# tsinghua-fib-lab/DRL-urban-planning

Measured on NVIDIA H100. Metric: ppo_update_graph_samples_per_sec, higher is better.
Workload: dtype f32

## Files before the change

drl_urban_planning_b200/csrc/sgnn_kernel.cuh:

```cuda
#pragma once
#include <cuda_runtime.h>
#include <math_constants.h>
#include <stdint.h>

#include "blob.h"
#include "layout.h"

namespace upb {

constexpr int NT = 512;
constexpr int NW = NT / 32;
constexpr int NS = 464;
constexpr int AS = 5632;
constexpr int KS = 160;
constexpr int CH = 96;
constexpr float MASK_FILL = -4294967296.0f;
constexpr float EPS_DEG = 1e-6f;

constexpr int S_WET = 0;
constexpr int S_BE = S_WET + 384;
constexpr int S_WPQ0 = S_BE + 16;
constexpr int S_B0 = S_WPQ0 + 512;
constexpr int S_WPQ1 = S_B0 + 16;
constexpr int S_B1 = S_WPQ1 + 512;
// ... 325 lines not shown
    v.z += __shfl_xor_sync(0xffffffffu, v.z, o); v.w += __shfl_xor_sync(0xffffffffu, v.w, o);
    w.x += __shfl_xor_sync(0xffffffffu, w.x, o); w.y += __shfl_xor_sync(0xffffffffu, w.y, o);
    w.z += __shfl_xor_sync(0xffffffffu, w.z, o); w.w += __shfl_xor_sync(0xffffffffu, w.w, o);
  }
  const int lane = threadIdx.x & 31, warp = threadIdx.x >> 5;
  if (lane < 4) { st4(red + warp * 20 + lane * 4, v); }
  __syncthreads();
  float keep = 0.f;
  if (threadIdx.x < 16) {
#pragma unroll
    for (int x = 0; x < NW; ++x) keep += red[x * 20 + threadIdx.x];
  }
  __syncthreads();
  if (lane < 4) { st4(red + warp * 20 + lane * 4, w); }
  if (threadIdx.x < 16) out32[threadIdx.x] = keep;
  __syncthreads();
  if (threadIdx.x < 16) {
    float s = 0.f;
#pragma unroll
    for (int x = 0; x < NW; ++x) s += red[x * 20 + threadIdx.x];
    out32[16 + threadIdx.x] = s;
  }
  __syncthreads();
}
__device__ __forceinline__ void block_sum_q4p1(float4 v, float sc1, float* red, float* out32) {
#pragma unroll
  for (int o = 4; o < 32; o <<= 1) {
    v.x += __shfl_xor_sync(0xffffffffu, v.x, o); v.y += __shfl_xor_sync(0xffffffffu, v.y, o);
    v.z += __shfl_xor_sync(0xffffffffu, v.z, o); v.w += __shfl_xor_sync(0xffffffffu, v.w, o);
  }
  sc1 = warp_sum(sc1);
  const int lane = threadIdx.x & 31, warp = threadIdx.x >> 5;
  if (lane < 4) st4(red + warp * 20 + lane * 4, v);
  if (lane == 0) red[warp * 20 + 16] = sc1;
  __syncthreads();
  if (threadIdx.x < 17) {
    float s = 0.f;
#pragma unroll
    for (int x = 0; x < NW; ++x) s += red[x * 20 + threadIdx.x];
    out32[threadIdx.x] = s;
  }
  __syncthreads();
}

template <bool TANH>
__device__ __forceinline__ void matvec8(const float* __restrict__ W, const float* __restrict__ b, int rows, int cols,
                                        const float* x, float* y) {
  const int p = threadIdx.x & 7;
  for (int row = threadIdx.x >> 3; row < rows; row += NT / 8) {
    const float* w = W + (size_t)row * cols;
    float acc = 0.f;
#pragma unroll 9
    for (int k = p; k < cols; k += 8) acc = fmaf(__ldg(w + k), x[k], acc);
    acc += __shfl_xor_sync(0xffffffffu, acc, 1);
    acc += __shfl_xor_sync(0xffffffffu, acc, 2);
    acc += __shfl_xor_sync(0xffffffffu, acc, 4);
    if (p == 0) {
      acc += __ldg(b + row);
      y[row] = TANH ? tanhf(acc) : acc;
    }
  }
}

__device__ __forceinline__ void load_weights(const float* __restrict__ P, float* sW) {
  const int t = threadIdx.x;
  static_assert(NT == 512, "load_weights is laid out for 512 threads");
  const int o = t >> 4, c = t & 15;
  const int src = o < 16 ? o * 32 + c : (o - 16) * 32 + 16 + c;
  const float wet = (t < 384 && (t >> 4) < F) ? __ldg(P + P_ENC_W + c * F + (t >> 4)) : 0.f;
  const float g0 = __ldg(P + P_GCN0_W + src), g1 = __ldg(P + P_GCN1_W + src);
  const float in0 = __ldg(P + P_MHA_IN_W + t), in1 = t < 256 ? __ldg(P + P_MHA_IN_W + 512 + t) : 0.f;
  float wq = 0.f, wk = 0.f, wv = 0.f, wo = 0.f;
  if (t < 256) {
    wq = __ldg(P + P_ATT_Q_W + t); wk = __ldg(P + P_ATT_K_W + t); wv = __ldg(P + P_ATT_V_W + t);
    wo = __ldg(P + P_MHA_OUT_W + t);
  }
  float lu[4];
#pragma unroll
  for (int j = 0; j < 4; ++j) lu[j] = __ldg(P + P_LU_W0 + t + NT * j);
  const float rd = __ldg(P + P_RD_W0 + t);
  float sm0 = 0.f, sm1 = 0.f, sm2 = 0.f;
  if (t < 16) { sm0 = __ldg(P + P_ENC_B + t); sm1 = __ldg(P + P_GCN0_B + t); sm2 = __ldg(P + P_GCN1_B + t); }
  else if (t < 32) { sm0 = __ldg(P + P_MHA_OUT_B + t - 16); sm1 = __ldg(P + P_ATT_Q_B + t - 16); sm2 = __ldg(P + P_ATT_V_B + t - 16); }
  else if (t < 64) { sm0 = __ldg(P + P_LU_B0 + t - 32); sm1 = __ldg(P + P_LU_W1 + t - 32); }
  else if (t < 96) { sm0 = __ldg(P + P_RD_B0 + t - 64); sm1 = __ldg(P + P_RD_W1 + t - 64); }
  else if (t < 112) { sm0 = __ldg(P + P_MHA_IN_B + t - 96); sm1 = __ldg(P + P_MHA_IN_B + 32 + t - 96); }

  float* tmp = sW + S_EPQ;
  if (t < 384) sW[S_WET + t] = wet;
  sW[S_WPQ0 + t] = g0; sW[S_WPQ1 + t] = g1;
  sW[S_WPQT0 + c * 32 + o] = g0; sW[S_WPQT1 + c * 32 + o] = g1;
  tmp[t] = in0;
  if (t < 256) {
    tmp[512 + t] = in1;
    tmp[768 + t] = wq; tmp[1024 + t] = wk; tmp[1280 + t] = wv;
    sW[S_WO + t] = wo;
    sW[S_WOT + c * 16 + o] = wo;
  }
#pragma unroll
  for (int j = 0; j < 4; ++j) sW[S_LUW0 + t + NT * j] = lu[j];
  sW[S_RDW0 + t] = rd;
  sW[S_RDW0T + c * 32 + o] = rd;
  if (t < 16) { sW[S_BE + t] = sm0; sW[S_B0 + t] = sm1; sW[S_B1 + t] = sm2; }
  else if (t < 32) { sW[S_BO + t - 16] = sm0; tmp[1536 + t - 16] = sm1; tmp[1552 + t - 16] = sm2; }
  else if (t < 64) { sW[S_LUB0 + t - 32] = sm0; sW[S_LUW1 + t - 32] = sm1; }
  else if (t < 96) { sW[S_RDB0 + t - 64] = sm0; sW[S_RDW1 + t - 64] = sm1; }
  else if (t < 112) { tmp[1568 + t - 96] = sm0; tmp[1584 + t - 96] = sm1; }
  __syncthreads();
  if (t < 256) {
    float q = 0.f, k = 0.f, v = 0.f;
#pragma unroll
    for (int m = 0; m < 16; ++m) {
      q = fmaf(tmp[o * 16 + m], tmp[768 + m * 16 + c], q);
      k = fmaf(tmp[(16 + o) * 16 + m], tmp[1024 + m * 16 + c], k);
      v = fmaf(tmp[(32 + o) * 16 + m], tmp[1280 + m * 16 + c], v);
    }
    sW[S_QC + t] = q; sW[S_KC + t] = k; sW[S_VC + t] = v;
    const int tr = c * 16 + o;
    sW[S_QCT + tr] = q; sW[S_KCT + tr] = k; sW[S_VCT + tr] = v;
  } else if (t < 272) {
    const int r = t - 256;
    float q = tmp[1568 + r], v = tmp[1584 + r];
#pragma unroll
    for (int m = 0; m < 16; ++m) {
      q = fmaf(tmp[r * 16 + m], tmp[1536 + m], q);
      v = fmaf(tmp[(32 + r) * 16 + m], tmp[1552 + m], v);
    }
    sW[S_QBC + r] = q;
    sW[S_VBC + r] = v;
  }
}

struct GraphView {
  int n, e, k, stage, gid;
  const float* x;
  float* H0g;
  float* H1g;
  float* EPQ;
  float* GPQ;
  float* H;
  float* inv;
  float* alpha;
  float* z;
  float* gz;
  float* ghead;
  const uint16_t* rp;
  const uint16_t* ord;
  int ord_rounds;
  const uint32_t* adj;
  const uint32_t* cuv;
  const int* cidx;
};

__device__ __forceinline__ uint32_t tf32_of(float x) {
  uint32_t r;
  asm("cvt.rna.tf32.f32 %0, %1;" : "=r"(r) : "f"(x));
  return r;
}
__device__ __forceinline__ void tf32_split(float x, uint32_t& hi, uint32_t& lo) {
  hi = tf32_of(x);
  lo = tf32_of(x - __uint_as_float(hi));
}
__device__ __forceinline__ void mma_tf32(float (&c)[4], uint32_t a0, uint32_t a1, uint32_t a2, uint32_t a3, uint32_t b0,
                                         uint32_t b1) {
  asm volatile("mma.sync.aligned.m16n8k8.row.col.f32.tf32.tf32.f32 {%0,%1,%2,%3}, {%4,%5,%6,%7}, {%8,%9}, {%0,%1,%2,%3};"
               : "+f"(c[0]), "+f"(c[1]), "+f"(c[2]), "+f"(c[3])
               : "r"(a0), "r"(a1), "r"(a2), "r"(a3), "r"(b0), "r"(b1));
}
#ifdef UPB_TILE_BF16
__device__ __forceinline__ uint32_t bf16_round(float x) {
  uint32_t u = __float_as_uint(x);
  u += 0x7fffu + ((u >> 16) & 1u);
  return u & 0xffff0000u;
}
__device__ __forceinline__ void mma_3x(float (&c)[4], float a0, float a1, float a2, float a3, uint32_t bh0, uint32_t bh1,
                                       uint32_t bl0, uint32_t bl1) {
  (void)bl0; (void)bl1;
  mma_tf32(c, bf16_round(a0), bf16_round(a1), bf16_round(a2), bf16_round(a3),
           bf16_round(__uint_as_float(bh0)), bf16_round(__uint_as_float(bh1)));
}
#else
__device__ __forceinline__ void mma_3x(float (&c)[4], float a0, float a1, float a2, float a3, uint32_t bh0, uint32_t bh1,
                                       uint32_t bl0, uint32_t bl1) {
  uint32_t h0, h1, h2, h3, l0, l1, l2, l3;
  tf32_split(a0, h0, l0); tf32_split(a1, h1, l1); tf32_split(a2, h2, l2); tf32_split(a3, h3, l3);
  mma_tf32(c, l0, l1, l2, l3, bh0, bh1);
  mma_tf32(c, h0, h1, h2, h3, bl0, bl1);
  mma_tf32(c, h0, h1, h2, h3, bh0, bh1);
}
#endif

__device__ __forceinline__ void gh_phase_tc(const GraphView& g, const float* Wpq, bool rescale) {
  const int lane = threadIdx.x & 31, warp = threadIdx.x >> 5;
  const int gq = lane >> 2, t = lane & 3;
  uint32_t bh[2][8], bl[2][8];
#pragma unroll
  for (int nt = 0; nt < 2; ++nt)
#pragma unroll
    for (int j = 0; j < 8; ++j) {
      const int k = (j < 4 ? 0 : 16) + 4 * t + (j & 3);
      tf32_split(Wpq[k * 16 + nt * 8 + gq], bh[nt][j], bl[nt][j]);
    }
  const int n = g.n;
  for (int m0 = warp * 16; m0 < n; m0 += NW * 16) {
    const int r0 = min(m0 + gq, n - 1), r1 = min(m0 + gq + 8, n - 1);
    const float4 v0 = ld4(g.GPQ + r0 * 32 + 4 * t), v1 = ld4(g.GPQ + r0 * 32 + 16 + 4 * t);
    const float4 w0 = ld4(g.GPQ + r1 * 32 + 4 * t), w1 = ld4(g.GPQ + r1 * 32 + 16 + 4 * t);
    const float rd0 = (float)(g.rp[r0 + 1] - g.rp[r0]) + EPS_DEG, rd1 = (float)(g.rp[r1 + 1] - g.rp[r1]) + EPS_DEG;
    float acc[2][4];
#pragma unroll
    for (int nt = 0; nt < 2; ++nt) {
      const float2 h0 = *reinterpret_cast<const float2*>(g.H + r0 * 16 + nt * 8 + 2 * t);
      const float2 h1 = *reinterpret_cast<const float2*>(g.H + r1 * 16 + nt * 8 + 2 * t);
      acc[nt][0] = h0.x * rd0; acc[nt][1] = h0.y * rd0; acc[nt][2] = h1.x * rd1; acc[nt][3] = h1.y * rd1;
      mma_3x(acc[nt], v0.x, w0.x, v0.y, w0.y, bh[nt][0], bh[nt][1], bl[nt][0], bl[nt][1]);
      mma_3x(acc[nt], v0.z, w0.z, v0.w, w0.w, bh[nt][2], bh[nt][3], bl[nt][2], bl[nt][3]);
      mma_3x(acc[nt], v1.x, w1.x, v1.y, w1.y, bh[nt][4], bh[nt][5], bl[nt][4], bl[nt][5]);
      mma_3x(acc[nt], v1.z, w1.z, v1.w, w1.w, bh[nt][6], bh[nt][7], bl[nt][6], bl[nt][7]);
    }
    const float s0 = rescale ? g.inv[r0] : 1.f, s1 = rescale ? g.inv[r1] : 1.f;
    __syncwarp();
#pragma unroll
    for (int nt = 0; nt < 2; ++nt) {
      if (m0 + gq < n)
        *reinterpret_cast<float2*>(g.H + (m0 + gq) * 16 + nt * 8 + 2 * t) = make_float2(acc[nt][0] * s0, acc[nt][1] * s0);
      if (m0 + gq + 8 < n)
        *reinterpret_cast<float2*>(g.H + (m0 + gq + 8) * 16 + nt * 8 + 2 * t) = make_float2(acc[nt][2] * s1, acc[nt][3] * s1);
    }
  }
}

template <bool RAW>
__device__ __forceinline__ int epq_phase(const GraphView& g, const float* hsrc, const float* WT, const float* b) {
  const int og = threadIdx.x & 7;
  const float4 bias = og < 4 ? ld4(b + og * 4) : f4(0.f);
  float2 wlo[16], whi[16];
#pragma unroll
  for (int c = 0; c < 16; ++c) {
    const float4 w = ld4(WT + c * 32 + og * 4);
    wlo[c] = make_float2(w.x, w.y); whi[c] = make_float2(w.z, w.w);
  }
  const int npair = (g.n + 1) >> 1;
  float amax = 0.f;
  for (int task = threadIdx.x; task < npair * 8; task += NT) {
    const int i0 = (task >> 3) * 2;
    const int i1 = min(i0 + 1, g.n - 1);
    float4 ha[4], hb[4];
#pragma unroll
    for (int j = 0; j < 4; ++j) { ha[j] = ld4(hsrc + i0 * 16 + j * 4); hb[j] = ld4(hsrc + i1 * 16 + j * 4); }
    float2 a0 = make_float2(bias.x, bias.y), a1 = make_float2(bias.z, bias.w), b0 = a0, b1 = a1;
#pragma unroll
    for (int c = 0; c < 16; ++c) {
      const float xa = comp(ha[c >> 2], c & 3), xb = comp(hb[c >> 2], c & 3);
      const float2 xa2 = make_float2(xa, xa), xb2 = make_float2(xb, xb);
      a0 = ffma2(wlo[c], xa2, a0); a1 = ffma2(whi[c], xa2, a1);
      b0 = ffma2(wlo[c], xb2, b0); b1 = ffma2(whi[c], xb2, b1);
    }
    amax = fmaxf(amax, fmaxf(fmaxf(fabsf(a0.x), fabsf(a0.y)), fmaxf(fabsf(a1.x), fabsf(a1.y))));
    amax = fmaxf(amax, fmaxf(fmaxf(fabsf(b0.x), fabsf(b0.y)), fmaxf(fabsf(b1.x), fabsf(b1.y))));
    if constexpr (RAW) {
      st4(g.EPQ + i0 * 32 + og * 4, make_float4(a0.x, a0.y, a1.x, a1.y));
      if (i1 != i0) st4(g.EPQ + i1 * 32 + og * 4, make_float4(b0.x, b0.y, b1.x, b1.y));
    } else {
      st4(g.EPQ + i0 * 32 + og * 4, make_float4(exp2a(a0.x), exp2a(a0.y), exp2a(a1.x), exp2a(a1.y)));
      if (i1 != i0) st4(g.EPQ + i1 * 32 + og * 4, make_float4(exp2a(b0.x), exp2a(b0.y), exp2a(b1.x), exp2a(b1.y)));
    }
  }
  return !(amax <= 10.9f) + !(amax <= 40.f);
}


template <int TIER, bool SM>
__device__ __forceinline__ void pull_forward(const GraphView& g, int q, bool save_h1, float* h1g, bool want_sums,
                                             float4& msum, float4& hsum) {
  const int odd = (threadIdx.x >> 2) & 1;
  const int offX = (odd ? 16 : 0) + q * 4, offY = (odd ? 0 : 16) + q * 4;
  const RowBase<SM> rX(g.EPQ + offX), rY(g.EPQ + offY);
  for (int task = threadIdx.x; task < g.ord_rounds * NT; task += NT) {
    const int i = g.ord[task >> 2];
    if (i == kNoNode) continue;
    const F2x2 A = rY.row((unsigned)i, 7), B = rX.row((unsigned)i, 7);
    const int beg = g.rp[i], end = g.rp[i + 1];
    float2 s0 = make_float2(0.f, 0.f), s1 = s0, s2 = s0, s3 = s0;
    int t = beg;
    for (; t + 1 < end; t += 2) {
      const unsigned k0 = g.adj[t] & 0xffffu, k1 = g.adj[t + 1] & 0xffffu;
      const F2x2 X0 = rX.row(k0, 7), Y0 = rY.row(k0, 7);
      const F2x2 X1 = rX.row(k1, 7), Y1 = rY.row(k1, 7);
      fwd_term<TIER>(A.a, B.a, Y0.a, X0.a, s0);
      fwd_term<TIER>(A.b, B.b, Y0.b, X0.b, s1);
      fwd_term<TIER>(A.a, B.a, Y1.a, X1.a, s2);
      fwd_term<TIER>(A.b, B.b, Y1.b, X1.b, s3);
    }
    if (t < end) {
      const unsigned k0 = g.adj[t] & 0xffffu;
      const F2x2 X0 = rX.row(k0, 7), Y0 = rY.row(k0, 7);
      fwd_term<TIER>(A.a, B.a, Y0.a, X0.a, s0);
      fwd_term<TIER>(A.b, B.b, Y0.b, X0.b, s1);
    }
    const float cnt = (float)(end - beg);
    const float4 acc = make_float4(cnt - (s0.x + s2.x), cnt - (s0.y + s2.y), cnt - (s1.x + s3.x), cnt - (s1.y + s3.y));
    const float iv = g.inv[i];
    float4 h = ld4(g.H + i * 16 + q * 4);
    h.x = fmaf(acc.x, iv, h.x); h.y = fmaf(acc.y, iv, h.y); h.z = fmaf(acc.z, iv, h.z); h.w = fmaf(acc.w, iv, h.w);
    st4(g.H + i * 16 + q * 4, h);
    if (save_h1) st4(h1g + i * 16 + q * 4, h);
    if (want_sums) { msum = msum + acc; hsum = hsum + h; }
  }
}

template <int TIER, bool SM>
__device__ __forceinline__ float4 pull_backward(const GraphView& g, int q, float4 ce4, bool use_head) {
  float4 bsum = f4(0.f);
  const float2 two = make_float2(2.f, 2.f);
// ... 298 lines not shown
}
__device__ __forceinline__ float half_sum(float v, unsigned mask) {
#pragma unroll
  for (int o = 8; o > 0; o >>= 1) v += __shfl_xor_sync(mask, v, o, 16);
  return v;
}

template <bool TRAIN>
__device__ __forceinline__ void softmax_seeds(const StepArgs& a, const BlobHeader& hd, const GraphView& g, float* sc,
                                              float* stats, int lane) {
  const int k = g.k, gid = g.gid;
  float lmax = -CUDART_INF_F;
  int lbest = 0x7fffffff;
  for (int j = lane; j < k; j += 32) {
    const float zj = g.z[j];
    if (zj > lmax) { lmax = zj; lbest = j; }
  }
#pragma unroll
  for (int o = 16; o > 0; o >>= 1) {
    const float om = __shfl_xor_sync(0xffffffffu, lmax, o);
    const int ob = __shfl_xor_sync(0xffffffffu, lbest, o);
    if (om > lmax || (om == lmax && ob < lbest)) { lmax = om; lbest = ob; }
  }
  const float zmax = lmax;
  float lsum = 0.f;
  for (int j = lane; j < k; j += 32) lsum += expf(g.z[j] - zmax);
  const float lse = zmax + logf(warp_sum(lsum));
  const int aidx = a.actions ? (int)sc[SC_ACT] : -1;
  float lent = 0.f;
  int slot = -1;
  for (int j = lane; j < k; j += 32) {
    const float lp = g.z[j] - lse;
    lent -= expf(lp) * lp;
    if (g.cidx[j] == aidx) slot = j;
  }
#pragma unroll
  for (int o = 16; o > 0; o >>= 1) slot = max(slot, __shfl_xor_sync(0xffffffffu, slot, o));
  float H = warp_sum(lent), logp = 0.f;
  int greedy = 0;
  if (k > 0) {
    greedy = g.cidx[lbest];
    if (a.actions) logp = slot >= 0 ? g.z[slot] - lse : MASK_FILL - lse;
  } else {
    H = 0.f;
    logp = 0.f;
  }
  const float V = sc[SC_VALUE];
  if (lane == 0) {
    sc[SC_LSE] = lse; sc[SC_ENT] = H; sc[SC_LOGP] = logp; sc[SC_SLOT] = (float)(slot + 1);
    if (a.out_value) a.out_value[gid] = V;
    if (a.out_logp) a.out_logp[gid] = logp;
    if (a.out_entropy) a.out_entropy[gid] = H;
    if (a.out_greedy) a.out_greedy[gid] = greedy;
  }
  if constexpr (!TRAIN) {
    if (a.uniforms != nullptr && a.out_sample != nullptr) {
      const float u = a.uniforms[gid];
      int pick = -1;
      if (k > 0) {
        const float S = warp_sum(lsum), target = u * S;
        float run = 0.f;
        int last = -1;
        for (int base = 0; base < k && pick < 0; base += 32) {
          const int j = base + lane;
          const float ej = j < k ? expf(g.z[j] - zmax) : 0.f;
          float c = ej;
#pragma unroll
          for (int o = 1; o < 32; o <<= 1) {
            const float t = __shfl_up_sync(0xffffffffu, c, o);
            if (lane >= o) c += t;
          }
          c += run;
          const unsigned pos = __ballot_sync(0xffffffffu, ej / S > 0.f);
          const unsigned hit = pos & __ballot_sync(0xffffffffu, c > target);
          if (hit) pick = base + __ffs(hit) - 1;
          if (pos) last = base + 31 - __clz(pos);
          run = __shfl_sync(0xffffffffu, c, 31);
        }
        if (pick < 0) pick = last;
        pick = g.cidx[pick];
      } else {
        const int cap = g.stage == 0 ? hd.e_cap : hd.n_cap;
        pick = min(cap - 1, max(0, (int)(u * (float)cap)));
      }
      if (lane == 0) a.out_sample[gid] = pick;
    }
  }
  if constexpr (TRAIN) {
    const float R = sc[SC_RET], dv = V - R;
    float glp = 0.f, gH = 0.f, surr = 0.f, negent = 0.f, in_ind = 0.f, kl = 0.f, clipped = 0.f;
    if (sc[SC_EXP] != 0.f) {
      in_ind = 1.f;
      const float dlp = logp - sc[SC_FLP];
      const float r = expf(dlp), A = sc[SC_ADV];
      const float lo = 1.f - a.clip_eps, hi = 1.f + a.clip_eps;
      const float s1 = r * A, s2 = fminf(fmaxf(r, lo), hi) * A;
      const bool inside = r >= lo && r <= hi;
      surr = -fminf(s1, s2);
      if (inside || s1 < s2) glp = -A * r * a.inv_ind;
      gH = -a.c_entropy * a.inv_ind;
      negent = -H;
      kl = expm1f(dlp) - dlp;
      clipped = inside ? 0.f : 1.f;
    }
    if (lane == 0) {
      sc[SC_GV] = 2.f * a.c_value * dv * a.inv_batch;
      gacc(stats, 0, dv * dv); gacc(stats, 1, surr); gacc(stats, 2, negent); gacc(stats, 3, 1.f); gacc(stats, 4, in_ind);
      gacc(stats, 5, g.stage == 0 ? 1.f : 0.f); gacc(stats, 6, g.stage == 1 ? 1.f : 0.f);
      gacc(stats, 7, (isfinite(V) && isfinite(logp) && isfinite(H)) ? 0.f : 1.f);
      if (a.diagnostics) {
        gacc(stats, 8, kl); gacc(stats, 9, clipped); gacc(stats, 10, R); gacc(stats, 11, R * R); gacc(stats, 12, dv);
      }
    }
    for (int j = lane; j < k; j += 32) {
      const float lp = g.z[j] - lse, p = expf(lp);
      g.gz[j] = glp * ((j == slot ? 1.f : 0.f) - p) - gH * p * (lp + H);
    }
  }
}

template <bool TRAIN>
__device__ __noinline__ void prefetch_next_graph(const StepArgs& a, int nitem) {
  const int T0 = threadIdx.x, TN = NT;
  const BlobHeader& hd = *reinterpret_cast<const BlobHeader*>(a.blob);
  const GraphDesc* descs = reinterpret_cast<const GraphDesc*>(a.blob + hd.off_desc);
  const int ng = a.ids ? a.ids[nitem] : nitem;
  const GraphDesc& nd = descs[ng];
  const char* px = reinterpret_cast<const char*>(a.blob + hd.off_x) + (size_t)nd.x_row * FS * 4;
  const char* pa = reinterpret_cast<const char*>(a.blob + hd.off_adj) + (size_t)nd.adj_off * 4;
  const char* pr = reinterpret_cast<const char*>(a.blob + hd.off_rowptr) + (size_t)nd.rp_off * 2;
  const char* po = reinterpret_cast<const char*>(a.blob + hd.off_order) + (size_t)nd.ord_off * 2;
  const int bx = nd.n * FS * 4, ba = nd.e * 8, br = (nd.n + 1) * 2, bo = nd.ord_rounds * NW * 16;
  for (int o = T0 * 128; o < bx; o += TN * 128) asm volatile("prefetch.global.L2 [%0];" ::"l"(px + o));
  for (int o = T0 * 128; o < ba; o += TN * 128) asm volatile("prefetch.global.L2 [%0];" ::"l"(pa + o));
  for (int o = T0 * 128; o < br; o += TN * 128) asm volatile("prefetch.global.L2 [%0];" ::"l"(pr + o));
  for (int o = T0 * 128; o < bo; o += TN * 128) asm volatile("prefetch.global.L2 [%0];" ::"l"(po + o));
  if (T0 >= TN - 32) {
    const int w = T0 - (TN - 32);
    const void* q = nullptr;
    if (w < 3) q = reinterpret_cast<const char*>(a.blob + hd.off_num) + (size_t)ng * NUMD * 4 + min(w * 128, NUMD * 4 - 4);
    else if (w < 5) q = reinterpret_cast<const char*>(a.blob + hd.off_cur) + (size_t)ng * FS * 4 + (w - 3) * (FS * 4 - 4);
    else if (w == 5) q = a.actions ? a.actions + (size_t)ng * 2 : nullptr;
    else if (TRAIN && w == 6) q = a.ret + ng;
    else if (TRAIN && w == 7) q = a.exps + ng;
    else if (TRAIN && w == 8) q = a.fixed_lp + ng;
    else if (TRAIN && w == 9) q = a.adv + ng;
    if (q) asm volatile("prefetch.global.L2 [%0];" ::"l"(q));
  }
}

template <bool SMEM>
__device__ __forceinline__ void gw_partial(const GraphView& g, const float* hin, int n, float* redbuf) {
  const int lane = threadIdx.x & 31, warp = threadIdx.x >> 5;
  const int to = lane >> 2, tc = lane & 3;
  float2 accp[4][2];
#pragma unroll
  for (int c = 0; c < 4; ++c) { accp[c][0] = make_float2(0.f, 0.f); accp[c][1] = make_float2(0.f, 0.f); }
  for (int i = warp; i < n; i += 8 * KW) {
    float4 gq[8], hv[8];
#pragma unroll
    for (int u = 0; u < 8; ++u) {
      const int ii = i + u * KW;
      if constexpr (SMEM) hv[u] = ii < n ? ld4(hin + ii * 16 + tc * 4) : f4(0.f);
      else hv[u] = ii < n ? __ldcg(reinterpret_cast<const float4*>(hin + (size_t)ii * 16 + tc * 4)) : f4(0.f);
    }
#pragma unroll
    for (int u = 0; u < 8; ++u) {
      const int ii = i + u * KW;
      gq[u] = ii < n ? ld4(g.GPQ + ii * 32 + to * 4) : f4(0.f);
    }
#pragma unroll
    for (int u = 0; u < 8; ++u) {
      const float2 g01 = make_float2(gq[u].x, gq[u].y), g23 = make_float2(gq[u].z, gq[u].w);
#pragma unroll
      for (int c = 0; c < 4; ++c) {
        const float hc_ = comp(hv[u], c);
        const float2 h2 = make_float2(hc_, hc_);
        accp[c][0] = ffma2(g01, h2, accp[c][0]);
        accp[c][1] = ffma2(g23, h2, accp[c][1]);
      }
    }
  }
#pragma unroll
  for (int x = 0; x < 4; ++x) {
    const int xp = x >> 1;
    st4(redbuf + warp * 512 + (to * 4 + x) * 16 + tc * 4,
        (x & 1) ? make_float4(accp[0][xp].y, accp[1][xp].y, accp[2][xp].y, accp[3][xp].y)
                : make_float4(accp[0][xp].x, accp[1][xp].x, accp[2][xp].x, accp[3][xp].x));
  }
}

#define UPB_STAMP(ID)                                                                      \
  do {                                                                                     \
    if (a.stamps != nullptr && blockIdx.x == 0 && threadIdx.x == 0 && first_item) a.stamps[ID] = clock64(); \
  } while (0)

#define UPB_WSTAMP()                                                                                         \
  do {                                                                                                       \
    if (a.stamps != nullptr && blockIdx.x == 0 && (threadIdx.x & 31) == 0 && first_item)                      \
      a.stamps[46 + (threadIdx.x >> 5)] = clock64();                                                         \
  } while (0)

#define UPB_WSTAMP_B()                                                                                       \
  do {                                                                                                       \
    if (a.stamps != nullptr && blockIdx.x == 0 && (threadIdx.x & 31) == 0 && first_item && threadIdx.x < 384) \
      a.stamps[212 + (threadIdx.x >> 5)] = clock64();                                                        \
  } while (0)

template <bool TRAIN, bool BIG>
__device__ void graph_body(const StepArgs& a, const BlobHeader& hd, const GraphDesc& d, int gid, float* smem,
                           float* gp, float* scr, bool first_item, uint64_t* mbar, unsigned mpar) {
  const int tid = threadIdx.x, lane = tid & 31, warp = tid >> 5;
  const int q = tid & 3;
  UPB_STAMP(0);
  float* sW = smem;
  float* sV = smem + S_VEC;
  float* sRed = smem + S_RED;
  float* sc = sV + V_SC;
  const float* P = a.params;

  GraphView g;
  g.n = d.n; g.e = d.e; g.k = d.k; g.stage = d.stage; g.gid = gid;
  g.x = reinterpret_cast<const float*>(a.blob + hd.off_x) + (size_t)d.x_row * FS;
  const float* gnum = reinterpret_cast<const float*>(a.blob + hd.off_num) + (size_t)gid * NUMD;
  const float* gcur = reinterpret_cast<const float*>(a.blob + hd.off_cur) + (size_t)gid * FS;
  const uint16_t* rp_g = reinterpret_cast<const uint16_t*>(a.blob + hd.off_rowptr) + d.rp_off;
  const uint16_t* ord_g = reinterpret_cast<const uint16_t*>(a.blob + hd.off_order) + d.ord_off;
  g.ord_rounds = d.ord_rounds;
  const uint32_t* adj_g = reinterpret_cast<const uint32_t*>(a.blob + hd.off_adj) + d.adj_off;
  const uint32_t* cuv_g = reinterpret_cast<const uint32_t*>(a.blob + hd.off_cand_uv) + d.cand_off;
  const int* cidx_g = reinterpret_cast<const int*>(a.blob + hd.off_cand_idx) + d.cand_off;
  const int n = g.n, e = g.e, k = g.k;
  g.H0g = scr;
  g.H1g = scr + (size_t)a.n_cap * 16;
  float* E0g = scr + (size_t)a.n_cap * 32;
  if constexpr (BIG) {
    float* b = scr + (size_t)a.n_cap * 64;
    g.EPQ = b;  b += (size_t)a.n_cap * 32;
    g.GPQ = b;  b += (size_t)a.n_cap * 32;
    g.H = b;    b += (size_t)a.n_cap * 16;
    g.inv = b;  b += a.n_cap;
    g.alpha = b; b += a.n_cap;
    const size_t kcap = (size_t)(a.e_cap > a.n_cap ? a.e_cap : a.n_cap);
    g.z = b;    b += kcap;
    g.gz = b;   b += kcap;
    g.ghead = b;
    g.rp = rp_g; g.adj = adj_g; g.cuv = cuv_g; g.cidx = cidx_g; g.ord = ord_g;
  } else {
    g.EPQ = smem + S_EPQ; g.GPQ = smem + S_GPQ; g.H = smem + S_H; g.inv = smem + S_INV;
    g.alpha = smem + S_ALPHA; g.z = smem + S_Z; g.gz = smem + S_GZ; g.ghead = smem + S_GHEAD;
    uint16_t* rp_s = reinterpret_cast<uint16_t*>(smem + S_RP);
    uint32_t* adj_s = reinterpret_cast<uint32_t*>(smem + S_ADJ);
    uint32_t* cuv_s = reinterpret_cast<uint32_t*>(smem + S_CUV);
    int* cidx_s = reinterpret_cast<int*>(smem + S_CIDX);
    if (tid == 0) {
      const unsigned b_rp = (unsigned)((n + 1 + 7) / 8) * 16u, b_ord = (unsigned)(d.ord_rounds * NW) * 16u;
      const unsigned b_adj = (unsigned)((2 * e + 3) / 4) * 16u, b_k = (unsigned)((k + 3) / 4) * 16u;
      const unsigned b_x = (unsigned)n * (FS * 4u);
      fence_proxy_async();
      mbar_expect_tx(mbar, b_rp + b_ord + b_adj + 2u * b_k + b_x);
      bulk_g2s(rp_s, rp_g, b_rp, mbar);
      if (b_ord) bulk_g2s(smem + S_ORD, ord_g, b_ord, mbar);
      if (b_adj) bulk_g2s(adj_s, adj_g, b_adj, mbar);
      if (b_k) { bulk_g2s(cuv_s, cuv_g, b_k, mbar); bulk_g2s(cidx_s, cidx_g, b_k, mbar); }
      bulk_g2s(smem + S_EPQ, g.x, b_x, mbar);
    }
    g.rp = rp_s; g.adj = adj_s; g.cuv = cuv_s; g.cidx = cidx_s;
    g.ord = reinterpret_cast<const uint16_t*>(smem + S_ORD);
  }
  float* vn = smem + S_GPQ;
  const float* psrc = nullptr;
  float* pdst = nullptr;
  if (tid < NUMD) { psrc = gnum + tid; pdst = sV + V_X52 + tid; }
  else if (tid >= 64 && tid < 64 + FS) { psrc = gcur + (tid - 64); pdst = sV + V_XCUR + (tid - 64); }
  else if (tid >= 96 && tid < 109) pdst = sc + (tid - 96);
  else if (tid == 109) { if (a.actions) { psrc = a.actions + ((size_t)gid * 2 + g.stage); pdst = sc + SC_ACT; } }
  else if (tid == 114) pdst = sc + SC_QUEUE;
  else if (TRAIN && tid == 110) { psrc = a.ret + gid; pdst = sc + SC_RET; }
  else if (TRAIN && tid == 111) { psrc = a.exps + gid; pdst = sc + SC_EXP; }
  else if (TRAIN && tid == 112) { psrc = a.fixed_lp + gid; pdst = sc + SC_FLP; }
  else if (TRAIN && tid == 113) { psrc = a.adv + gid; pdst = sc + SC_ADV; }
  const float pval = psrc ? __ldg(psrc) : 0.f;
  stage_vn_weights(P, vn);
  if (pdst) *pdst = pval;
  if constexpr (!BIG) mbar_wait(mbar, mpar);
  __syncthreads();
  UPB_STAMP(1);

  numeric_l0(vn, sV + V_X52, sV + V_A0, tid);
  for (int i = tid; i < n; i += NT) g.inv[i] = 1.0f / ((float)(g.rp[i + 1] - g.rp[i]) + EPS_DEG);
  if constexpr (BIG) {
    for (int task = tid; task < n * 4; task += NT) {
      const int i = task >> 2;
      const float* xr = g.x + (size_t)i * FS;
      float4 xv[6];
#pragma unroll
      for (int f4i = 0; f4i < 6; ++f4i) xv[f4i] = __ldg(reinterpret_cast<const float4*>(xr) + f4i);
      float4 acc = ld4(sW + S_BE + q * 4);
#pragma unroll
      for (int f4i = 0; f4i < 6; ++f4i) {
#pragma unroll
        for (int j = 0; j < 4; ++j) {
          const float xs = comp(xv[f4i], j);
          const float4 w = ld4(sW + S_WET + (f4i * 4 + j) * 16 + q * 4);
          acc.x = fmaf(w.x, xs, acc.x); acc.y = fmaf(w.y, xs, acc.y);
          acc.z = fmaf(w.z, xs, acc.z); acc.w = fmaf(w.w, xs, acc.w);
        }
      }
      st4(g.H + i * 16 + q * 4, acc);
      if (TRAIN) st4(g.H0g + i * 16 + q * 4, acc);
    }
  } else {
    const int c2 = (lane & 7) * 2;
    float2 w[24];
#pragma unroll
    for (int f = 0; f < 24; ++f) w[f] = *reinterpret_cast<const float2*>(sW + S_WET + f * 16 + c2);
    const float2 be = *reinterpret_cast<const float2*>(sW + S_BE + c2);
    const float* xs = smem + S_EPQ;
    for (int i = warp * 4 + (lane >> 3); i < n; i += NW * 4) {
      const float4* xr = reinterpret_cast<const float4*>(xs + i * FS);
      float2 acc = be;
#pragma unroll
      for (int f4i = 0; f4i < 6; ++f4i) {
        const float4 xv = xr[f4i];
        acc = ffma2(w[f4i * 4 + 0], make_float2(xv.x, xv.x), acc);
        acc = ffma2(w[f4i * 4 + 1], make_float2(xv.y, xv.y), acc);
        acc = ffma2(w[f4i * 4 + 2], make_float2(xv.z, xv.z), acc);
        acc = ffma2(w[f4i * 4 + 3], make_float2(xv.w, xv.w), acc);
      }
      *reinterpret_cast<float2*>(g.H + i * 16 + c2) = acc;
      if (TRAIN) *reinterpret_cast<float2*>(g.H0g + i * 16 + c2) = acc;
    }
  }
  if (warp == NW - 1 && lane < 16) {
    float s = sW[S_BE + lane];
#pragma unroll
    for (int f = 0; f < F; ++f) s = fmaf(sW[S_WET + f * 16 + lane], sV[V_XCUR + f], s);
    sV[V_HC + lane] = s;
  }
  __syncthreads();
  UPB_STAMP(2);
// ... 251 lines not shown
        const float gs = ai * (dp - gdot);
        gsh = gsh + h * gs;
        st4(g.H + i * 16 + q * 4, (gmn4 + gh4 * ai + qk4 * gs) * g.inv[i]);
      }
    }
  }
  __syncthreads();
  UPB_STAMP(13);
  if (g.stage == 0) {
    if (tid < 512) {
      const int r_ = tid >> 4, c_ = tid & 15;
      const float G = sV[V_GWEFF + tid], hc = sV[V_HC + c_], gc = sV[V_GC + r_];
      const int o = P_LU_W0 + r_ * 64 + c_;
      gacc(gp, o, G);
      gacc(gp, o + 16, gc * hc);
      gacc(gp, o + 32, G * hc);
      gacc(gp, o + 48, G - gc * hc);
    }
    if (tid < 32) { gacc(gp, P_LU_B0 + tid, sV[V_GC + tid]); gacc(gp, P_LU_W1 + tid, sV[V_GW2 + tid]); }
    if (warp == 1) {
      const int c = lane & 15, r0 = (lane >> 4) * 16;
      float s0 = 0.f, s1 = 0.f;
#pragma unroll
      for (int r = 0; r < 16; ++r) {
        const float* w = sW + S_LUW0 + (r0 + r) * 64;
        s0 = fmaf(w[16 + c] - w[48 + c], sV[V_GC + r0 + r], s0);
        s1 = fmaf(w[32 + c], sV[V_GWEFF + (r0 + r) * 16 + c], s1);
      }
      float s = s0 + s1;
      s += __shfl_xor_sync(0xffffffffu, s, 16);
      if (lane < 16) sV[V_GHC + c] = s;
    }
  } else {
    if (tid < 512) gacc(gp, P_RD_W0 + tid, sV[V_GWEFF + tid]);
    if (tid < 32) { gacc(gp, P_RD_B0 + tid, sV[V_GC + tid]); gacc(gp, P_RD_W1 + tid, sV[V_GW2 + tid]); }
  }

  block_sum_q4(gsh, sRed, sV + V_GSH);
  if (warp == 0) {
    const int c = lane & 15;
    float s = 0.f;
#pragma unroll
    for (int j = 0; j < 16; ++j) s = fmaf(sW[S_KCT + j * 16 + c], sV[V_GSH + j], s);
    const float gqp = 0.25f * s;
    float t = sV[V_GHC + c];
#pragma unroll
    for (int r = 0; r < 16; ++r) t = fmaf(sW[S_QC + r * 16 + c], __shfl_sync(0xffffffffu, gqp, r), t);
    __syncwarp();
    if (lane < 16) { sV[V_GHC + c] = t; sV[V_GQP + c] = gqp; }
  }
  if (g.stage == 1) {
    for (int task = tid; task < k * 16; task += NT) {
      const int j = task >> 4, c = task & 15;
      const int node = (int)g.cuv[j];
      g.H[node * 16 + c] += g.ghead[(size_t)j * 16 + c] * g.inv[node];
    }
  }
  __syncthreads();
  UPB_STAMP(14);
  if (tid < 256) {
    const int r = tid >> 4, cc = tid & 15;
    gacc(gp, G_QC + tid, sV[V_GQP + r] * sV[V_HC + cc]);
    gacc(gp, G_KC + tid, 0.25f * sV[V_QP + r] * sV[V_GSH + cc]);
    gacc(gp, G_VC + tid, sV[V_GVP + r] * sV[V_HBAR + cc]);
    gacc(gp, P_MHA_OUT_W + tid, sV[V_GSV + 48 + r] * sV[V_VP + cc]);
  } else if (tid < 272) {
    const int c = tid - 256;
    gacc(gp, G_QBC + c, sV[V_GQP + c]);
    gacc(gp, G_VBC + c, sV[V_GVP + c]);
    gacc(gp, P_MHA_OUT_B + c, sV[V_GSV + 48 + c]);
  }

  for (int l = 1; l >= 0; --l) {
    const float* Wpq = sW + (l == 0 ? S_WPQ0 : S_WPQ1);
    const float* hin = l == 0 ? g.H0g : g.H1g;
    int tier = tier_last;
    if (l == 0) {
      if constexpr (BIG) {
#pragma unroll 2
        for (int i = tid; i < n * 8; i += NT) st4(g.EPQ + i * 4, __ldcg(reinterpret_cast<const float4*>(E0g) + i));
      } else {
        if (tid == 0) {
          fence_proxy_async();
          mbar_expect_tx(mbar + 1, (unsigned)n * 128u);
          bulk_g2s(g.EPQ, E0g, (unsigned)n * 128u, mbar + 1);
        }
        mbar_wait(mbar + 1, mpar);
      }
      tier = tier_first;
      __syncthreads();
      UPB_STAMP(17);
    }
    const bool last = (l == 1);
    const float4 ce4 = last ? ld4(sV + V_CE + q * 4) : f4(0.f);
    const bool use_head = last && g.stage == 0;
    const float4 bsum = tier == 2 ? pull_backward<2, false>(g, q, ce4, use_head)
                        : tier ? pull_backward<1, false>(g, q, ce4, use_head) : pull_backward<0, false>(g, q, ce4, use_head);
    block_sum_q4(bsum, sRed, sV + V_TMP16);
    UPB_STAMP(15+(1-l)*3);
    bool hin_smem = false;
    if constexpr (!BIG) {
      hin_smem = n <= HIN_NODES;
      if (tid == 0) {
        fence_proxy_async();
        if (hin_smem) {
          mbar_expect_tx(mbar + 3, (unsigned)n * 64u);
          bulk_g2s(smem + S_EPQ + KW * 512, hin, (unsigned)n * 64u, mbar + 3);
        }
        if (l == 0 && n <= XEARLY_NODES) {
          mbar_expect_tx(mbar + 2, (unsigned)n * (FS * 4u));
          bulk_g2s(smem + S_Z, g.x, (unsigned)n * (FS * 4u), mbar + 2);
        }
      }
    }
    if (tid < 16) gacc(gp, (l == 0 ? P_GCN0_B : P_GCN1_B) + tid, sV[V_TMP16 + tid]);
    gh_phase_tc(g, Wpq, l == 1);
    if (hin_smem) mbar_wait(mbar + 3, l == 1 ? 0u : 1u);
    if (warp < KW) {
      if (hin_smem) gw_partial<true>(g, smem + S_EPQ + KW * 512, n, smem + S_EPQ);
      else gw_partial<false>(g, hin, n, smem + S_EPQ);
    }
    __syncthreads();
    if (tid < 512) {
      const float* redbuf = smem + S_EPQ;
      float s = 0.f;
#pragma unroll
      for (int w = 0; w < KW; ++w) s += redbuf[w * 512 + tid];
      const int o = tid >> 4, c = tid & 15;
      const int dst = o < 16 ? o * 32 + c : (o - 16) * 32 + 16 + c;
      gacc(gp, (l == 0 ? P_GCN0_W : P_GCN1_W) + dst, s);
    }
    __syncthreads();
    UPB_STAMP(16+(1-l)*3);
  }

  {
    float* redbuf = smem + S_GPQ;
    const float* xsrc = g.x;
    if constexpr (!BIG) {
      if (n <= XEARLY_NODES) {
        xsrc = smem + S_Z;
      } else {
        if (tid == 0) {
          fence_proxy_async();
          mbar_expect_tx(mbar + 2, (unsigned)n * (FS * 4u));
          bulk_g2s(smem + S_EPQ, g.x, (unsigned)n * (FS * 4u), mbar + 2);
        }
        xsrc = smem + S_EPQ;
      }
    }
    float4 hs = f4(0.f);
    for (int task = tid; task < n * 4; task += NT) hs = hs + ld4(g.H + (task >> 2) * 16 + q * 4);
    if constexpr (!BIG) { mbar_wait(mbar + 2, mpar); __syncthreads(); }
    const int tcc = lane / 6, tf = lane % 6;
    float2 accp[4][2];
#pragma unroll
    for (int f = 0; f < 4; ++f) { accp[f][0] = make_float2(0.f, 0.f); accp[f][1] = make_float2(0.f, 0.f); }
    if (lane < 24) {
      for (int i = warp; i < n; i += 4 * NW) {
        float4 gh[4], xv[4];
#pragma unroll
        for (int u = 0; u < 4; ++u) {
          const int ii = i + u * NW;
          const bool ok = ii < n;
          if constexpr (BIG) xv[u] = ok ? __ldg(reinterpret_cast<const float4*>(xsrc + (size_t)ii * FS) + tf) : f4(0.f);
          else xv[u] = ok ? ld4(xsrc + ii * FS + tf * 4) : f4(0.f);
          gh[u] = ok ? ld4(g.H + ii * 16 + tcc * 4) : f4(0.f);
        }
#pragma unroll
        for (int u = 0; u < 4; ++u) {
          const float2 g01 = make_float2(gh[u].x, gh[u].y), g23 = make_float2(gh[u].z, gh[u].w);
#pragma unroll
          for (int f = 0; f < 4; ++f) {
            const float xf = comp(xv[u], f);
            const float2 x2 = make_float2(xf, xf);
            accp[f][0] = ffma2(g01, x2, accp[f][0]);
            accp[f][1] = ffma2(g23, x2, accp[f][1]);
          }
        }
      }
#pragma unroll
      for (int x = 0; x < 4; ++x) {
        const int xp = x >> 1;
        st4(redbuf + warp * 384 + (tcc * 4 + x) * 24 + tf * 4,
            (x & 1) ? make_float4(accp[0][xp].y, accp[1][xp].y, accp[2][xp].y, accp[3][xp].y)
                    : make_float4(accp[0][xp].x, accp[1][xp].x, accp[2][xp].x, accp[3][xp].x));
      }
    }
    block_sum_q4(hs, sRed, sV + V_TMP16);
    if (tid < 384) {
      const int c = tid / 24, f = tid % 24;
      if (f < F) {
        float s = sV[V_GHC + c] * sV[V_XCUR + f];
#pragma unroll
        for (int w = 0; w < NW; ++w) s += redbuf[w * 384 + tid];
        gacc(gp, P_ENC_W + c * F + f, s);
      }
    }
    if (tid < 16) gacc(gp, P_ENC_B + tid, sV[V_TMP16 + tid] + sV[V_GHC + tid]);
  }
  __syncthreads();
  UPB_STAMP(21);
}


constexpr int MAX_PEERS = 16;
constexpr int SLICE = 128;
constexpr int NSLICE = G_ROW / SLICE;
static_assert(G_ROW % SLICE == 0, "slices tile the gradient row");
constexpr int CHAIN_S0 = G_QC / SLICE;
constexpr int CHAIN_S1 = (G_STATS - 1) / SLICE;
constexpr int FLAG_STRIDE = 128;
constexpr size_t XCHG_FLAGS = (size_t)2 * MAX_PEERS * G_ROW;
constexpr size_t XCHG_FLOATS = XCHG_FLAGS + (size_t)2 * MAX_PEERS * FLAG_STRIDE;
static_assert(NSLICE <= FLAG_STRIDE, "one flag word per slice");
static_assert(NSLICE == 114 && CHAIN_S0 == 107 && CHAIN_S1 == 113,
              "tests/test_gpu_shapes.py runs the fused tail at grids of 113 / 114 / 115 CTAs around NSLICE: move them");
constexpr unsigned PEER_SPIN_LIMIT = 1u << 24;

__device__ __forceinline__ float ld_relaxed(const float* p, bool sys) {
  float v;
  if (sys) asm volatile("ld.relaxed.sys.global.f32 %0, [%1];" : "=f"(v) : "l"(p));
  else asm volatile("ld.relaxed.gpu.global.f32 %0, [%1];" : "=f"(v) : "l"(p));
  return v;
}
__device__ __forceinline__ void st_relaxed(float* p, float v, bool sys) {
  if (sys) asm volatile("st.relaxed.sys.global.f32 [%0], %1;" ::"l"(p), "f"(v) : "memory");
  else asm volatile("st.relaxed.gpu.global.f32 [%0], %1;" ::"l"(p), "f"(v) : "memory");
}
__device__ __forceinline__ unsigned ld_acquire(const unsigned* p, bool sys) {
  unsigned v;
  if (sys) asm volatile("ld.acquire.sys.global.u32 %0, [%1];" : "=r"(v) : "l"(p) : "memory");
  else asm volatile("ld.acquire.gpu.global.u32 %0, [%1];" : "=r"(v) : "l"(p) : "memory");
  return v;
}
__device__ __forceinline__ void st_release(unsigned* p, unsigned v, bool sys) {
  if (sys) asm volatile("st.release.sys.global.u32 [%0], %1;" ::"l"(p), "r"(v) : "memory");
  else asm volatile("st.release.gpu.global.u32 [%0], %1;" ::"l"(p), "r"(v) : "memory");
}

__device__ __forceinline__ void grid_arrive(unsigned int* ctr) {
  __syncthreads();
  if (threadIdx.x == 0) {
    __threadfence();
    atomicAdd(ctr, 1u);
  }
}
__device__ __forceinline__ void grid_wait(unsigned int* ctr, unsigned int target) {
  if (threadIdx.x == 0) {
    unsigned int v;
    do {
      asm volatile("ld.acquire.gpu.global.u32 %0, [%1];" : "=r"(v) : "l"(ctr) : "memory");
    } while ((int)(v - target) < 0);
    __threadfence();
  }
  __syncthreads();
}

__device__ __forceinline__ void adam_elem(const StepArgs& a, int i, float g, float m, float v, float p, float step_size,
                                          float bc2_sqrt) {
  const float w1 = 1.f - a.beta1, w2 = 1.f - a.beta2;
  if (a.weight_decay != 0.f) g = __fmaf_rn(a.weight_decay, p, g);
  m = __fadd_rn(m, __fmul_rn(w1, __fsub_rn(g, m)));
  v = __fadd_rn(__fmul_rn(v, a.beta2), __fmul_rn(__fmul_rn(w2, g), g));
  const float denom = __fadd_rn(__fdiv_rn(__fsqrt_rn(v), bc2_sqrt), a.adam_eps);
  a.params_rw[i] = __fadd_rn(p, __fmul_rn(-step_size, __fdiv_rn(m, denom)));
  a.adam_m[i] = m;
  a.adam_v[i] = v;
}

__device__ void fused_tail(const StepArgs& a, float* smem, unsigned stage_bits) {
  const int tid = threadIdx.x;
  const int nparts = gridDim.x;
  const int world = a.world, me = a.rank;
  const bool sys = world > 1;
  const unsigned par = a.seq & 1u;
  const bool chain_cta = blockIdx.x == gridDim.x - 1;
  __shared__ float sh_adam[12];
  __shared__ long long sh_steps[6];
  __shared__ unsigned sh_bits;
  __shared__ int sh_timeout;
  __shared__ float* sh_push[MAX_PEERS];
#define UPB_TSTAMP(ID) do { if (a.stamps != nullptr && blockIdx.x == 0 && threadIdx.x == 0) a.stamps[ID] = clock64(); } while (0)
  UPB_TSTAMP(40);
  float* const mine = a.peers[me];
  const float* const pull = mine + (size_t)par * MAX_PEERS * G_ROW;
  const unsigned* const myflags = reinterpret_cast<const unsigned*>(mine + XCHG_FLAGS) + (size_t)par * MAX_PEERS * FLAG_STRIDE;
  if (tid < world) sh_push[tid] = a.peers[tid] + ((size_t)par * MAX_PEERS + me) * G_ROW;
  if (tid == 32) { sh_timeout = 0; sh_bits = 0u; }
  if (tid == 0 && stage_bits) atomicOr(a.gridbar + 2 + par, stage_bits);
  if (tid == 1 && blockIdx.x == 0) a.gridbar[2 + (par ^ 1u)] = 0u;
  if (tid < 6) {
    const int seg = tid >> 1, live = tid & 1;
    const long long stp = a.steps_in[1 + seg] + live;
    const double bc1 = 1.0 - ipow((double)a.beta1, stp > 0 ? stp : 1);
    const double bc2 = 1.0 - ipow((double)a.beta2, stp > 0 ? stp : 1);
    sh_adam[tid * 2 + 0] = (float)((double)a.lr / bc1);
    sh_adam[tid * 2 + 1] = (float)sqrt(bc2);
    sh_steps[tid] = stp;
  }
  const int col0 = blockIdx.x * SLICE + (tid >> 2), part = tid & 3;
  const bool attn0 = (col0 >= P_MHA_IN_W && col0 < P_MHA_OUT_W) || (col0 >= P_ATT_Q_W && col0 < P_LU_W0);
  const bool real0 = part == 0 && col0 < NUM_PARAMS && !attn0;
  float pm = 0.f, pv = 0.f, pp = 0.f;
  if (real0) { pm = a.adam_m[col0]; pv = a.adam_v[col0]; pp = a.params_rw[col0]; }
  float* sG = smem;
  float* sWin = sG + 816;
  float* sW3 = sWin + 768;
  float* sB = sW3 + 768;
  float* sOut = sB + 48;
  const int pW[3] = {P_ATT_Q_W, P_ATT_K_W, P_ATT_V_W};
  const int pB[3] = {P_ATT_Q_B, P_ATT_K_B, P_ATT_V_B};
  float cm[4], cv[4], cp[4];
  int cdst[4];
  if (chain_cta) {
    const float* P = a.params_rw;
    for (int i = tid; i < 768; i += NT) sWin[i] = P[P_MHA_IN_W + i];
    if (tid < 256) { sW3[tid] = P[P_ATT_Q_W + tid]; sW3[256 + tid] = P[P_ATT_K_W + tid]; sW3[512 + tid] = P[P_ATT_V_W + tid]; }
    if (tid < 16) { sB[tid] = P[P_ATT_Q_B + tid]; sB[16 + tid] = P[P_ATT_K_B + tid]; sB[32 + tid] = P[P_ATT_V_B + tid]; }
#pragma unroll
    for (int j = 0; j < 4; ++j) {
      const int i = tid + j * NT;
      int dst = 0;
      if (i < 768) dst = pW[i >> 8] + (i & 255);
      else if (i < 1536) dst = P_MHA_IN_W + (i - 768);
      else if (i < 1584) dst = pB[(i - 1536) >> 4] + ((i - 1536) & 15);
      else if (i < 1632) dst = P_MHA_IN_B + (i - 1584);
      cdst[j] = dst;
      if (i < 1632) { cm[j] = a.adam_m[dst]; cv[j] = a.adam_v[dst]; cp[j] = P[dst]; }
    }
  }
  grid_arrive(a.gridbar);
  grid_wait(a.gridbar, a.bar_target);
  UPB_TSTAMP(41);
  unsigned mybits;
  asm volatile("ld.acquire.gpu.global.u32 %0, [%1];" : "=r"(mybits) : "l"(a.gridbar + 2 + par) : "memory");
  const unsigned flagword = (a.seq << 2) | (mybits & 3u);

  float* sPart = smem + 4096;
// ... 219 lines not shown
```

Measured before the change: 1.711 million.

## Move graph weight-gradient reductions from packed FFMA2 to split-TF32 MMA

Two outer-product reductions over graph nodes, in gw_partial and the encoder weight gradient, are rewritten from per-lane FFMA2 accumulation to m16n8k8 TF32 mma.sync with hi/lo operand splitting (3xTF32), which keeps accuracy close to FP32. The goal is to offload the reduction FLOPs from CUDA cores to tensor cores and to cut the FMA instruction count. tf32_split now leaves the low part unrounded, which saves one cvt per split. Operand loads become narrower and strided (float2 and scalar gathers), which may raise shared and global load instruction counts, and the extra MMAs and splits add overhead for small node counts.

```diff
diff --git a/drl_urban_planning_b200/csrc/sgnn_kernel.cuh b/drl_urban_planning_b200/csrc/sgnn_kernel.cuh
--- a/drl_urban_planning_b200/csrc/sgnn_kernel.cuh
+++ b/drl_urban_planning_b200/csrc/sgnn_kernel.cuh
@@ -501,14 +501,9 @@
   const int* cidx;
 };
 
-__device__ __forceinline__ uint32_t tf32_of(float x) {
-  uint32_t r;
-  asm("cvt.rna.tf32.f32 %0, %1;" : "=r"(r) : "f"(x));
-  return r;
-}
 __device__ __forceinline__ void tf32_split(float x, uint32_t& hi, uint32_t& lo) {
-  hi = tf32_of(x);
-  lo = tf32_of(x - __uint_as_float(hi));
+  asm("cvt.rna.tf32.f32 %0, %1;" : "=r"(hi) : "f"(x));
+  lo = __float_as_uint(x - __uint_as_float(hi));
 }
 __device__ __forceinline__ void mma_tf32(float (&c)[4], uint32_t a0, uint32_t a1, uint32_t a2, uint32_t a3, uint32_t b0,
                                          uint32_t b1) {
@@ -1113,41 +1108,47 @@
 template <bool SMEM>
 __device__ __forceinline__ void gw_partial(const GraphView& g, const float* hin, int n, float* redbuf) {
   const int lane = threadIdx.x & 31, warp = threadIdx.x >> 5;
-  const int to = lane >> 2, tc = lane & 3;
-  float2 accp[4][2];
-#pragma unroll
-  for (int c = 0; c < 4; ++c) { accp[c][0] = make_float2(0.f, 0.f); accp[c][1] = make_float2(0.f, 0.f); }
-  for (int i = warp; i < n; i += 8 * KW) {
-    float4 gq[8], hv[8];
-#pragma unroll
-    for (int u = 0; u < 8; ++u) {
-      const int ii = i + u * KW;
-      if constexpr (SMEM) hv[u] = ii < n ? ld4(hin + ii * 16 + tc * 4) : f4(0.f);
-      else hv[u] = ii < n ? __ldcg(reinterpret_cast<const float4*>(hin + (size_t)ii * 16 + tc * 4)) : f4(0.f);
-    }
-#pragma unroll
-    for (int u = 0; u < 8; ++u) {
-      const int ii = i + u * KW;
-      gq[u] = ii < n ? ld4(g.GPQ + ii * 32 + to * 4) : f4(0.f);
-    }
-#pragma unroll
-    for (int u = 0; u < 8; ++u) {
-      const float2 g01 = make_float2(gq[u].x, gq[u].y), g23 = make_float2(gq[u].z, gq[u].w);
-#pragma unroll
-      for (int c = 0; c < 4; ++c) {
-        const float hc_ = comp(hv[u], c);
-        const float2 h2 = make_float2(hc_, hc_);
-        accp[c][0] = ffma2(g01, h2, accp[c][0]);
-        accp[c][1] = ffma2(g23, h2, accp[c][1]);
+  const int gq = lane >> 2, t = lane & 3;
+  float acc[2][2][4];
+#pragma unroll
+  for (int mt = 0; mt < 2; ++mt)
+#pragma unroll
+    for (int nt = 0; nt < 2; ++nt)
+#pragma unroll
+      for (int q = 0; q < 4; ++q) acc[mt][nt][q] = 0.f;
+  for (int kc = warp; kc * 8 < n; kc += 2 * KW) {
+    float4 ga[2][2];
+    float2 hb[2][2];
+#pragma unroll
+    for (int u = 0; u < 2; ++u)
+#pragma unroll
+      for (int s = 0; s < 2; ++s) {
+        const int i = (kc + u * KW) * 8 + s * 4 + t;
+        const bool ok = i < n;
+        if constexpr (SMEM) hb[u][s] = ok ? *reinterpret_cast<const float2*>(hin + i * 16 + 2 * gq) : make_float2(0.f, 0.f);
+        else hb[u][s] = ok ? __ldcg(reinterpret_cast<const float2*>(hin + (size_t)i * 16 + 2 * gq)) : make_float2(0.f, 0.f);
+        ga[u][s] = ok ? ld4(g.GPQ + i * 32 + 4 * gq) : f4(0.f);
+      }
+#pragma unroll
+    for (int u = 0; u < 2; ++u) {
+      uint32_t bh[2][2], bl[2][2];
+#pragma unroll
+      for (int s = 0; s < 2; ++s) {
+        tf32_split(hb[u][s].x, bh[0][s], bl[0][s]);
+        tf32_split(hb[u][s].y, bh[1][s], bl[1][s]);
+      }
+#pragma unroll
+      for (int nt = 0; nt < 2; ++nt) {
+        mma_3x(acc[0][nt], ga[u][0].x, ga[u][0].y, ga[u][1].x, ga[u][1].y, bh[nt][0], bh[nt][1], bl[nt][0], bl[nt][1]);
+        mma_3x(acc[1][nt], ga[u][0].z, ga[u][0].w, ga[u][1].z, ga[u][1].w, bh[nt][0], bh[nt][1], bl[nt][0], bl[nt][1]);
       }
     }
   }
 #pragma unroll
   for (int x = 0; x < 4; ++x) {
-    const int xp = x >> 1;
-    st4(redbuf + warp * 512 + (to * 4 + x) * 16 + tc * 4,
-        (x & 1) ? make_float4(accp[0][xp].y, accp[1][xp].y, accp[2][xp].y, accp[3][xp].y)
-                : make_float4(accp[0][xp].x, accp[1][xp].x, accp[2][xp].x, accp[3][xp].x));
+    const int mt = x >> 1, r = 2 * (x & 1);
+    st4(redbuf + warp * 512 + (gq * 4 + x) * 16 + t * 4,
+        make_float4(acc[mt][0][r], acc[mt][1][r], acc[mt][0][r + 1], acc[mt][1][r + 1]));
   }
 }
 
@@ -1705,39 +1706,43 @@
     float4 hs = f4(0.f);
     for (int task = tid; task < n * 4; task += NT) hs = hs + ld4(g.H + (task >> 2) * 16 + q * 4);
     if constexpr (!BIG) { mbar_wait(mbar + 2, mpar); __syncthreads(); }
-    const int tcc = lane / 6, tf = lane % 6;
-    float2 accp[4][2];
-#pragma unroll
-    for (int f = 0; f < 4; ++f) { accp[f][0] = make_float2(0.f, 0.f); accp[f][1] = make_float2(0.f, 0.f); }
-    if (lane < 24) {
-      for (int i = warp; i < n; i += 4 * NW) {
-        float4 gh[4], xv[4];
-#pragma unroll
-        for (int u = 0; u < 4; ++u) {
-          const int ii = i + u * NW;
-          const bool ok = ii < n;
-          if constexpr (BIG) xv[u] = ok ? __ldg(reinterpret_cast<const float4*>(xsrc + (size_t)ii * FS) + tf) : f4(0.f);
-          else xv[u] = ok ? ld4(xsrc + ii * FS + tf * 4) : f4(0.f);
-          gh[u] = ok ? ld4(g.H + ii * 16 + tcc * 4) : f4(0.f);
-        }
-#pragma unroll
-        for (int u = 0; u < 4; ++u) {
-          const float2 g01 = make_float2(gh[u].x, gh[u].y), g23 = make_float2(gh[u].z, gh[u].w);
-#pragma unroll
-          for (int f = 0; f < 4; ++f) {
-            const float xf = comp(xv[u], f);
-            const float2 x2 = make_float2(xf, xf);
-            accp[f][0] = ffma2(g01, x2, accp[f][0]);
-            accp[f][1] = ffma2(g23, x2, accp[f][1]);
+    {
+      const int gq = lane >> 2, t = lane & 3;
+      float acc[3][4];
+#pragma unroll
+      for (int nt = 0; nt < 3; ++nt)
+#pragma unroll
+        for (int q = 0; q < 4; ++q) acc[nt][q] = 0.f;
+      for (int kc = warp; kc * 8 < n; kc += 2 * NW) {
+        float2 ha[2][2];
+        float xb[2][2][3];
+#pragma unroll
+        for (int u = 0; u < 2; ++u)
+#pragma unroll
+          for (int s = 0; s < 2; ++s) {
+            const int i = (kc + u * NW) * 8 + s * 4 + t;
+            const bool ok = i < n;
+            ha[u][s] = ok ? *reinterpret_cast<const float2*>(g.H + i * 16 + 2 * gq) : make_float2(0.f, 0.f);
+#pragma unroll
+            for (int nt = 0; nt < 3; ++nt) {
+              if constexpr (BIG) xb[u][s][nt] = ok ? __ldg(xsrc + (size_t)i * FS + nt * 8 + gq) : 0.f;
+              else xb[u][s][nt] = ok ? xsrc[i * FS + nt * 8 + gq] : 0.f;
+            }
           }
-        }
-      }
-#pragma unroll
-      for (int x = 0; x < 4; ++x) {
-        const int xp = x >> 1;
-        st4(redbuf + warp * 384 + (tcc * 4 + x) * 24 + tf * 4,
-            (x & 1) ? make_float4(accp[0][xp].y, accp[1][xp].y, accp[2][xp].y, accp[3][xp].y)
-                    : make_float4(accp[0][xp].x, accp[1][xp].x, accp[2][xp].x, accp[3][xp].x));
+#pragma unroll
+        for (int u = 0; u < 2; ++u)
+#pragma unroll
+          for (int nt = 0; nt < 3; ++nt) {
+            uint32_t bh0, bl0, bh1, bl1;
+            tf32_split(xb[u][0][nt], bh0, bl0);
+            tf32_split(xb[u][1][nt], bh1, bl1);
+            mma_3x(acc[nt], ha[u][0].x, ha[u][0].y, ha[u][1].x, ha[u][1].y, bh0, bh1, bl0, bl1);
+          }
+      }
+#pragma unroll
+      for (int nt = 0; nt < 3; ++nt) {
+        *reinterpret_cast<float2*>(redbuf + warp * 384 + (2 * gq) * 24 + nt * 8 + 2 * t) = make_float2(acc[nt][0], acc[nt][1]);
+        *reinterpret_cast<float2*>(redbuf + warp * 384 + (2 * gq + 1) * 24 + nt * 8 + 2 * t) = make_float2(acc[nt][2], acc[nt][3]);
       }
     }
     block_sum_q4(hs, sRed, sV + V_TMP16);
```

Measured after the change: 1.764 million (median of 6 runs). +3.1%, better.
